# dbdexter-dev/meteor_demod

Measured on AMD Instinct MI355X. Metric: IQ Msamples/s demodulated (whole node), higher is better.
Workload: dtype f32

## Files before the change

### meteor_demod_amd/csrc/demod_device.h

```cpp
#ifndef MDEMOD_DEVICE_H
#define MDEMOD_DEVICE_H

#include <hip/hip_runtime.h>
#include <stdint.h>

#include "pll_flags.h"

#pragma clang fp contract(off)

#define MD_TWO_PI_D 6.283185307179586476925286766559
#define MD_HALF_PI_D 1.5707963267948966192313216916398
#define MD_TWO_PI_F 6.28318548202514648437500f
#define MD_PI_F     3.14159274101257324218750f

struct cf32 { float re, im; };

__device__ __forceinline__ bool md_any(bool p) { return __builtin_amdgcn_ballot_w64(p) != 0ull; }
__device__ __forceinline__ bool md_all(bool p) { return __builtin_amdgcn_ballot_w64(!p) == 0ull; }

template <typename T>
__device__ __forceinline__ T md_lane_select(uint64_t mask, T a, T b)
{
	static_assert(sizeof(T) == 4, "one 32-bit register");
	T r;
// ... 157 lines not shown
	x.re = x.re - bias_re;
	x.im = x.im - bias_im;
	x.re = x.re * gain;
	x.im = x.im * gain;
	return x;
}

template <bool SHORT = false>
__device__ __forceinline__ void
md_agc_gain(cf32 scaled, float &gain)
{
	const float mag = SHORT ? md_cabsf_short(scaled.re, scaled.im) : md_cabsf(scaled.re, scaled.im);
	gain = gain + 0.0001f * (190.0f - mag);
	gain = (0.0f > gain) ? 0.0f : gain;
}

__device__ __forceinline__ float
md_agc_gain_step(float gain, float mag)
{
	gain = gain + 0.0001f * (190.0f - mag);
	return (0.0f > gain) ? 0.0f : gain;
}

template <bool SHORT = false>
__device__ __forceinline__ cf32
md_agc(cf32 x, float &gain, float &bias_re, float &bias_im)
{
	x = md_agc_apply(x, gain, bias_re, bias_im);
	md_agc_gain<SHORT>(x, gain);
	return x;
}

#define MD_TWO_PI_LO (-0x1.777a5cp-23f)

template <bool F32 = false>
__device__ __forceinline__ void
md_nco_advance(float &phase, float freq)
{
	phase = phase + freq;
	if (F32) {
		const float w = (phase - MD_TWO_PI_F) - MD_TWO_PI_LO;
		phase = (phase >= MD_TWO_PI_F) ? w : phase;
	} else if (phase >= MD_TWO_PI_F)
		phase = (float)((double)phase - MD_TWO_PI_D);
}

#define MD_FOUR_PI_F 12.56637096405029296875f
__device__ __forceinline__ float
md_wrap_2pi(float xf)
{
	const bool wraps = !(fabsf(xf) < MD_TWO_PI_F);
	const float once = (xf < 0.0f) ? (xf + MD_TWO_PI_F) + MD_TWO_PI_LO : (xf - MD_TWO_PI_F) - MD_TWO_PI_LO;
	float r = wraps ? once : xf;
	const bool far = !(fabsf(xf) < MD_FOUR_PI_F);
	if (__builtin_expect(md_any(far), 0)) {
		if (far) r = (float)fmod((double)xf, MD_TWO_PI_D);
	}
	return r;
}

__device__ __forceinline__ float
md_wrap_2pi_near(float xf, bool &far)
{
	const bool wraps = !(fabsf(xf) < MD_TWO_PI_F);
	const float once = (xf < 0.0f) ? (xf + MD_TWO_PI_F) + MD_TWO_PI_LO : (xf - MD_TWO_PI_F) - MD_TWO_PI_LO;
	far = !(fabsf(xf) < MD_FOUR_PI_F);
	return wraps ? once : xf;
}
__device__ __forceinline__ float md_wrap_2pi_far(float xf) { return (float)fmod((double)xf, MD_TWO_PI_D); }

__device__ __forceinline__ float
md_tanh_lut(const float *lut, float v)
{
	const float c = __builtin_amdgcn_fmed3f(v, -16.0f, 15.0f);
	return lut[(int)c + 16];
}

__device__ __forceinline__ float
md_tanh_lut_uniform(const float *lut, float v)
{
	float t = (v >= 15.0f) ? 1.0f : -1.0f;
	if (__builtin_expect(md_any(v > -16.0f && v < 15.0f), 0)) t = md_tanh_lut(lut, v);
	return t;
}

__device__ __forceinline__ void
md_tanh_lut_uniform2(const float *lut, float a, float b, float &ta, float &tb)
{
	ta = (a >= 15.0f) ? 1.0f : -1.0f;
	tb = (b >= 15.0f) ? 1.0f : -1.0f;
	if (__builtin_expect(md_any((a > -16.0f && a < 15.0f) || (b > -16.0f && b < 15.0f)), 0)) {
		ta = md_tanh_lut(lut, a);
// ... 67 lines not shown
		if (__builtin_expect((m_lock_event | m_turn) != 0ull, 0)) {
			const PllFlagStep s = pll_flags_step(fl, md_lane_bit(m_below), md_lane_bit(m_above),
			                                     p.freq >= fmax ? PLL_FREQ_HIGH : (p.freq <= -fmax ? PLL_FREQ_LOW : PLL_FREQ_INSIDE));
			fl = s.fl; first = s.first; changed = s.changed;
		}
		p.freq = md_clamp_sym(p.freq, fmax);
		return changed;
	}

	const uint32_t below = (p.err < 85.0f) ? 1u : 0u, above = (p.err > 105.0f) ? 1u : 0u;
	const uint32_t lock_now = below & (fl ^ 1u);
	const uint32_t unlock_now = above & fl;
	const uint32_t lock2 = lock_now + lock_now;
	first = lock2 ^ (lock2 & fl);
	fl = fl | lock_now | lock2;
	fl = fl ^ (fl & unlock_now);

	if (!(fl & 1u)) p.freq = (float)((double)p.freq + ((fl & 4u) ? 0.000001 : -0.000001));
	fl = (p.freq >= fmax) ? (fl & ~4u) : ((p.freq <= -fmax) ? (fl | 4u) : fl);
	p.freq = md_clamp_sym(p.freq, fmax);
	return lock_now | unlock_now;
}

__device__ __forceinline__ uint64_t
md_pll_update_common(PllWord &p, uint32_t fl, const float *lut, float alpha, float beta, float fmax, float i, float q, float &ph, bool &far)
{
	const float ti = md_tanh_lut(lut, i), tq = md_tanh_lut(lut, q);
	const float e = ti * q - tq * i;

	ph = p.phase + alpha * e;
	p.phase = md_wrap_2pi_near(ph, far);
	p.freq = p.freq + beta * e;

	const float decayed = p.err * (1.0f - 0.001f);
	p.err = (float)((double)decayed + fabs((double)e) * (double)0.001f);

	const uint64_t m_below = __builtin_amdgcn_ballot_w64(p.err < 85.0f), m_above = __builtin_amdgcn_ballot_w64(p.err > 105.0f);
	const uint64_t m_locked = __builtin_amdgcn_ballot_w64((fl & 1u) != 0);
	const uint64_t m_lock_event = (m_below & ~m_locked) | (m_above & m_locked);
	const float swept = (float)((double)p.freq + ((fl & 4u) ? 0.000001 : -0.000001));
	p.freq = md_lane_select(m_locked ^ m_lock_event, swept, p.freq);
	const uint64_t m_turn = __builtin_amdgcn_ballot_w64(fabsf(p.freq) >= fmax);
	return m_lock_event | m_turn;
}

__device__ __forceinline__ uint32_t
md_pll_update_rare(const PllWord &p, uint32_t &fl, float fmax, uint32_t &first)
{
	const PllFlagStep s = pll_flags_step(fl, p.err < 85.0f ? 1u : 0u, p.err > 105.0f ? 1u : 0u,
	                                     p.freq >= fmax ? PLL_FREQ_HIGH : (p.freq <= -fmax ? PLL_FREQ_LOW : PLL_FREQ_INSIDE));
	fl = s.fl; first = s.first;
	return s.changed;
}

// ... 25 lines not shown
```

### meteor_demod_amd/csrc/demod_kernel_gat.hip

```cpp
#include "rotwin_body.h"
#include "hip_host.h"

namespace {

typedef float gpair_t __attribute__((ext_vector_type(2)));
typedef float gquad_t __attribute__((ext_vector_type(4)));
typedef __attribute__((address_space(3))) const gquad_t lds_gquad;
typedef __attribute__((address_space(3))) const float lds_gfloat;

template <int FMT> struct GFmt;
template <> struct GFmt<16> {
	enum { G = 4 };
	__device__ static __forceinline__ gpair_t get(const uint4 &q, int k) { const uint32_t w = (&q.x)[k]; return gpair_t{ (float)(int)(int16_t)(w & 0xFFFFu), (float)((int)w >> 16) }; }
	__device__ static __forceinline__ gpair_t one(uint32_t w) { return gpair_t{ (float)(int)(int16_t)(w & 0xFFFFu), (float)((int)w >> 16) }; }
};
template <> struct GFmt<8> {
	enum { G = 8 };
	__device__ static __forceinline__ gpair_t get(const uint4 &q, int k) { const uint32_t w = (&q.x)[k >> 1] >> (16 * (k & 1)); return gpair_t{ (float)((int)(w & 0xFFu) - 128), (float)((int)((w >> 8) & 0xFFu) - 128) }; }
	__device__ static __forceinline__ gpair_t one(uint16_t w) { return gpair_t{ (float)((int)(w & 0xFFu) - 128), (float)((int)(w >> 8) - 128) }; }
};
template <> struct GFmt<32> {
	enum { G = 2 };
	__device__ static __forceinline__ gpair_t get(const uint4 &q, int k) { return gpair_t{ __uint_as_float((&q.x)[2 * k]), __uint_as_float((&q.x)[2 * k + 1]) }; }
	__device__ static __forceinline__ gpair_t one(float2 w) { return gpair_t{ w.x, w.y }; }
};

template <int KT, int FMT>
struct WinG {
	static constexpr int G = GFmt<FMT>::G, kTaps = KT, kBack = KT - 1, AMAX = G - 1, NS = KT + AMAX, NW = 4 * ((NS + 3) / 4), SLIDE = 4, MAXSL = 1, DEPTH = 1,
	                     BLOCK = MDEMOD_RW_BLOCK, ROTN = 1, RING = 32, REGSLOTS = 0;
	static constexpr bool GATHER = true, SCALAR_SLIDE = false, VCONST = false;
	static constexpr bool LOCK_EARLY_OUT = true;
	static constexpr bool RARE_ONE_BRANCH = false;
	static_assert(NS % G == 0 && NS / G <= 36, "whole 16-byte loads, and few enough of them to stay in registers");
	typedef typename RFmt<FMT>::sample_t sample_t;
	__device__ __forceinline__ void setup(uint32_t) {}
	__device__ static __forceinline__ void put_history(const float2 *, bool, int) {}
	__device__ static __forceinline__ void put_init(const RGran<FMT> (&)[1], int) {}
	__device__ static __forceinline__ void put(const RGran<FMT> (&)[1], int) {}
	__device__ static __forceinline__ void fir(uint32_t, int, int, const DemodConsts &, int, float &, float &) {}

	__device__ static __forceinline__ void
	fir_gather(uint32_t ctab_addr, const sample_t *src, const float2 *hist, int v, int n, int bank, const DemodConsts &C, float &re, float &im)
	{
		const int oldest = v - kBack - (KT - 1);
		const int d = oldest & (G - 1);
		const int start = oldest - d;
		const int o = AMAX - d;
		const uint32_t row = ctab_addr + 4u * (uint32_t)(__mul24(bank * 4 + (o & 3), C.ctab_row_stride) + (o & ~3));
		gpair_t acc = { 0.0f, 0.0f };
		if (__builtin_expect(md_all(start >= 0 && start + NS <= n), 1)) {
			uint4 raw[NS / G];
#pragma unroll
			for (int g = 0; g < NS / G; g++) __builtin_memcpy(&raw[g], src + start + G * g, 16);
#pragma unroll
			for (int s4 = 0; s4 < NS / 4; s4++) {
// ... 74 lines not shown
```

### meteor_demod_amd/csrc/demod_kernel_rot.hip

```cpp
#include "rotwin_body.h"
#include "rot_fir_bounds.h"
#include "hip_host.h"
#ifdef ROTWIN_ASM_HEADER
#include ROTWIN_ASM_HEADER
#else
#include "rotwin_asm.h"
#endif

namespace {

static_assert(ROTWIN_NCH * 8 == 80 && ROTWIN_SLIDE == 8, "window = ten chunks of eight, a slide brings one");


__device__ __forceinline__ void
rot_fir(uint32_t row_addr, int rot, int flags, float &re, float &im)
{
	int tmp;
#if ROTWIN_PK == 1 || ROTWIN_PK == 3
	typedef float pair_t __attribute__((ext_vector_type(2)));
	pair_t acc, p0, p1;
	asm volatile(ROTWIN_FIR_ASM
	             : [acc] "=&v"(acc), [p0] "=&v"(p0), [p1] "=&v"(p1), [tmp] "=&s"(tmp)
	             : [addr] "v"(row_addr), [rot] "s"(rot), [flags] "s"(flags)
	             : "vcc", "scc", ROTWIN_COEF_CLOBBERS);
// ... 33 lines not shown
{
	int tmp;
	asm volatile(ROTWIN_PUT_F32_ASM
	             : [tmp] "=&s"(tmp), [rot] "+s"(q), [base] "+s"(base)
	             : [f0] "v"(f[0]), [f1] "v"(f[1]), [f2] "v"(f[2]), [f3] "v"(f[3]), [f4] "v"(f[4]), [f5] "v"(f[5]), [f6] "v"(f[6]), [f7] "v"(f[7]),
	               [f8] "v"(f[8]), [f9] "v"(f[9]), [f10] "v"(f[10]), [f11] "v"(f[11]), [f12] "v"(f[12]), [f13] "v"(f[13]), [f14] "v"(f[14]), [f15] "v"(f[15])
	             : "vcc", "scc", "v255", "memory");
}
__device__ __forceinline__ void
rot_put_floats(const uint32_t (&f)[16], int q)
{
	int base = 0;
	rot_put_floats(f, q, base);
}
template <> __device__ __forceinline__ void
rot_put<32>(const RGran<32> &a, const RGran<32> &b, int &q, int &base)
{
	uint32_t f[16];
#pragma unroll
	for (int i = 0; i < 8; i++) { f[i] = a.w[i]; f[8 + i] = b.w[i]; }
	rot_put_floats(f, q, base);
}

template <int FMT, int COMPACT = 0, int BLK = MDEMOD_RW_BLOCK, int VC = 0, int RSL = 0>
struct WinF {
	static constexpr int kTaps = 65, kBack = 64, NW = 80, SLIDE = 8, AMAX = NW - kTaps, MAXSL = 1, DEPTH = 1, BLOCK = BLK, ROTN = NW / SLIDE, RING = 32;
	static constexpr bool GATHER = false;
	static constexpr bool SCALAR_SLIDE = true;
	static constexpr bool VCONST = VC != 0;
	static_assert(SLIDE == ROTWIN_SLIDE && ROTN == ROTWIN_NCH, "the slide's assembly counts for itself");
	__device__ __forceinline__ void setup(uint32_t) {}
	static constexpr int REGSLOTS = RSL;
	static constexpr bool LOCK_EARLY_OUT = true;
	static constexpr bool RARE_ONE_BRANCH = true;
	__device__ static __forceinline__ void put_history(const float2 *hist, bool valid, int q)
	{
		const uint4 *h4 = reinterpret_cast<const uint4 *>(hist);
		uint32_t f[16];
#pragma unroll
		for (int i = 0; i < 4; i++) {
			uint4 h = h4[i];
			if (!valid) h = make_uint4(0, 0, 0, 0);
			f[4 * i] = h.x; f[4 * i + 1] = h.y; f[4 * i + 2] = h.z; f[4 * i + 3] = h.w;
		}
		rot_put_floats(f, q);
	}
	__device__ static __forceinline__ void put(const RGran<FMT> (&g)[2], int q) { int base = 0; rot_put<FMT>(g[0], g[1], q, base); }
	__device__ static __forceinline__ void put_init(const RGran<FMT> (&g)[2], int q) { put(g, q); }
	__device__ static __forceinline__ void slide(const RGran<FMT> (&g)[2], int &rot, int &base) { rot_put<FMT>(g[0], g[1], rot, base); }
	__device__ static __forceinline__ void fir(uint32_t ctab_addr, int a, int bank, const DemodConsts &C, int rot, float &re, float &im)
	{
		const int o = AMAX - a;
		uint32_t row_addr;
		if (COMPACT) row_addr = rot_mad24((uint32_t)(bank * 4 + (o & 3)), 4u * (uint32_t)C.ctab_row_stride, ctab_addr + 4u * (uint32_t)(o & ~3));
		else row_addr = rot_mad24(rot_mad24((uint32_t)a, (uint32_t)C.interp, (uint32_t)bank), 4u * (uint32_t)C.ctab_row_stride, ctab_addr);
		static_assert(AMAX == 15, "two bits of a / 4");
		const uint64_t ex = __builtin_amdgcn_ballot_w64(true);
		const RotFirQ q = rot_fir_q(ex, __builtin_amdgcn_ballot_w64(a >= 4), __builtin_amdgcn_ballot_w64(a >= 8), __builtin_amdgcn_ballot_w64(a >= 12));
		int q_hi = q.q_hi;
		asm("" : "+s"(q_hi));
		const int flags = rot_fir_flags(q.q_lo, q_hi);
#ifdef ROT_EXP_NOSKIP
		int f0 = __builtin_amdgcn_readfirstlane(flags);
		asm volatile("s_and_b32 %0, %0, 0" : "+s"(f0) : : "scc");
		rot_fir(row_addr, rot, f0, re, im);
#else
		rot_fir(row_addr, rot, flags, re, im);
#endif
	}
};

typedef float pair_t2 __attribute__((ext_vector_type(2)));

template <int NA>
__device__ __forceinline__ void
rot_fir_acc(uint32_t addr, int rot, int last, pair_t2 &acc)
{
	int tmp;
// ... 28 lines not shown
	else
		asm volatile(ROTWIN_MIGRATE5_ASM : [tmp] "=&s"(tmp) : ROT_F16_OPERANDS, [rot] "s"(q) : "vcc", "scc", "v255", ROTWIN_ACC_CLOBBERS, "memory");
}
template <int NA>
__device__ __forceinline__ void
rot_put_acc(const uint32_t (&f)[16], int q)
{
	int tmp;
	if constexpr (NA == 10)
		asm volatile(ROTWIN_PUT_ACC_ASM : [tmp] "=&s"(tmp) : ROT_F16_OPERANDS, [rot] "s"(q) : "vcc", "scc", ROTWIN_ACC_CLOBBERS, "memory");
	else if constexpr (NA == 2)
		asm volatile(ROTWIN_PUT_ACC2_ASM : [tmp] "=&s"(tmp) : ROT_F16_OPERANDS, [rot] "s"(q) : "vcc", "scc", ROTWIN_ACC_CLOBBERS, "memory");
	else
		asm volatile(ROTWIN_PUT_ACC5_ASM : [tmp] "=&s"(tmp) : ROT_F16_OPERANDS, [rot] "s"(q) : "vcc", "scc", ROTWIN_ACC_CLOBBERS, "memory");
}

template <int BLK, int NA, int MSL>
struct WinH {
	static constexpr int NR = 10, SLIDE = 8, NW = SLIDE * (NR + NA), kTaps = NA == 10 ? 129 : 65, kBack = kTaps - 1, AMAX = NW - kTaps, MAXSL = MSL, DEPTH = MSL,
	                     BLOCK = BLK, ROTN = NR, RING = 32, REGSLOTS = 0;
	static constexpr bool GATHER = false, SCALAR_SLIDE = false, VCONST = false;
	static constexpr bool LOCK_EARLY_OUT = true;
	static constexpr bool RARE_ONE_BRANCH = false;
	static_assert((NA == 10 || NA == 2 || NA == 5) && AMAX == (NA == 5 ? 55 : 31) && kBack % SLIDE == 0, "wide (160 slots, 129 taps), mid (96 slots, 65 taps) or far (120 slots, 65 taps)");
	__device__ __forceinline__ void setup(uint32_t) {}
	__device__ static __forceinline__ void place(const uint32_t (&f)[16], int c)
	{
		if (c < NR) rot_put_floats(f, c);
		else rot_put_acc<NA>(f, c - NR);
	}
	__device__ static __forceinline__ void put_history(const float2 *hist, bool valid, int c)
	{
		const uint4 *h4 = reinterpret_cast<const uint4 *>(hist);
		uint32_t f[16];
#pragma unroll
		for (int i = 0; i < 4; i++) {
			uint4 h = h4[i];
			if (!valid) h = make_uint4(0, 0, 0, 0);
			f[4 * i] = h.x; f[4 * i + 1] = h.y; f[4 * i + 2] = h.z; f[4 * i + 3] = h.w;
		}
		place(f, c);
	}
	__device__ static __forceinline__ void put_init(const RGran<32> (&g)[2], int c)
	{
		uint32_t f[16];
#pragma unroll
// ... 99 lines not shown
```

### meteor_demod_amd/csrc/demod_kernel_rotp.hip

```cpp
#include "rotwin_body.h"
#include "hip_host.h"
#ifdef ROTPK_ASM_HEADER
#include ROTPK_ASM_HEADER
#else
#include "rotpk_asm.h"
#endif

namespace {

typedef float pair_t __attribute__((ext_vector_type(2)));

template <int GEO> struct GeoP;
#ifndef ROTP_WIDE_DEPTH
#define ROTP_WIDE_DEPTH 1
#endif
#ifndef ROTP_MID_DEPTH
#define ROTP_MID_DEPTH 1
#endif
#ifndef ROTP_FAR_DEPTH
#define ROTP_FAR_DEPTH 2
#endif
template <> struct GeoP<0> { static constexpr int kTaps = 129, NW = MDEMOD_RW_WIDE_NW, MAXSL = 1, DEPTH = ROTP_WIDE_DEPTH, BLOCK = MDEMOD_RW_WIDE_BLOCK; };
template <> struct GeoP<1> { static constexpr int kTaps = 65, NW = MDEMOD_RW_MID_NW, MAXSL = 1, DEPTH = ROTP_MID_DEPTH, BLOCK = MDEMOD_RW_BLOCK; };
#ifndef ROTP_FAR_MAXSL
// ... 37 lines not shown
		               [g7] "v"(g[7]), [g8] "v"(g[8]), [g9] "v"(g[9]), [g10] "v"(g[10]), [g11] "v"(g[11]), [g12] "v"(g[12]),  \
		               [g13] "v"(g[13]), [g14] "v"(g[14]), [g15] "v"(g[15]), [rot] "s"(q)                                     \
		             : "vcc", "scc", "v255", "memory");                                                                       \
	}
#define ROTP_PUT8(GEO, NAME)                                                                                                  \
	__device__ __forceinline__ void AsmP<GEO, 8>::put(const uint32_t (&g)[8], int q)                                          \
	{                                                                                                                         \
		int tmp;                                                                                                              \
		asm volatile(ROTPK_##NAME##_8_PUT_ASM                                                                                 \
		             : [tmp] "=&s"(tmp)                                                                                       \
		             : [g0] "v"(g[0]), [g1] "v"(g[1]), [g2] "v"(g[2]), [g3] "v"(g[3]), [g4] "v"(g[4]), [g5] "v"(g[5]), [g6] "v"(g[6]),  \
		               [g7] "v"(g[7]), [rot] "s"(q)                                                                           \
		             : "vcc", "scc", "v255", "memory");                                                                       \
	}
ROTP_PUT16(0, WIDE) ROTP_PUT16(1, MID) ROTP_PUT16(2, FAR) ROTP_PUT8(0, WIDE) ROTP_PUT8(1, MID) ROTP_PUT8(2, FAR)

template <int GEO, int FMT>
struct WinP {
	static constexpr int kTaps = GeoP<GEO>::kTaps, kBack = kTaps - 1, NW = GeoP<GEO>::NW, SLIDE = 16, AMAX = NW - kTaps,
	                     MAXSL = GeoP<GEO>::MAXSL, DEPTH = GeoP<GEO>::DEPTH, BLOCK = GeoP<GEO>::BLOCK, NCH = NW / SLIDE, GD = FMT == 16 ? 16 : 8, REGSLOTS = 0, ROTN = NCH, RING = 32;
	static constexpr bool GATHER = false, SCALAR_SLIDE = false, VCONST = false;
	static constexpr bool LOCK_EARLY_OUT = true;
	static constexpr bool RARE_ONE_BRANCH = false;
	__device__ __forceinline__ void setup(uint32_t) {}
	static_assert(kBack % SLIDE == 0 && NW % SLIDE == 0, "history and window are whole chunks");

	__device__ static __forceinline__ void put_history(const float2 *hist, bool valid, int q)
	{
		uint32_t g[GD];
#pragma unroll
		for (int k = 0; k < 16; k++) {
			float2 h = hist[k];
			if (!valid) h = make_float2(0.0f, 0.0f);
			if (FMT == 16) {
				g[k] = ((uint32_t)(int)h.x & 0xFFFFu) | ((uint32_t)(int)h.y << 16);
			} else {
				const uint32_t s = (uint32_t)(((int)h.x + 128) & 0xFF) | ((uint32_t)(((int)h.y + 128) & 0xFF) << 8);
				if (k & 1) g[k / 2] |= s << 16; else g[k / 2] = s;
			}
		}
		AsmP<GEO, FMT>::put(g, q);
	}
	__device__ static __forceinline__ void put(const RGran<FMT> (&gr)[4], int q)
	{
		uint32_t g[GD];
#pragma unroll
// ... 65 lines not shown
```

### meteor_demod_amd/csrc/rot_firing_index.h

```cpp
#ifndef MDEMOD_ROT_FIRING_INDEX_H
#define MDEMOD_ROT_FIRING_INDEX_H

#include <stdint.h>

#if defined(__HIPCC__) || defined(__CUDACC__)
#define ROT_IDX_HD __host__ __device__
#else
#define ROT_IDX_HD
#endif


ROT_IDX_HD constexpr bool
rot_ring_geometry_ok(uint32_t ring, uint32_t block)
{
	return (ring == 16u || ring == 32u) && (block == 256u || block == 512u);
}

ROT_IDX_HD constexpr uint32_t
rot_ring_group_bytes(uint32_t block)
{
	return block * 16u;
}

ROT_IDX_HD constexpr uint32_t
// ... 27 lines not shown
}


enum { ROT_CLOCK_ROW_SHIFT = 6 };

ROT_IDX_HD constexpr uint32_t
rot_clock_sel(bool c1, bool c2, bool c3)
{
	return c1 ? 0u : (c2 ? 16u : (c3 ? 32u : 48u));
}

ROT_IDX_HD constexpr int32_t
rot_clock_entry_scaled(int32_t isub)
{
	return (int32_t)((uint32_t)isub << ROT_CLOCK_ROW_SHIFT);
}

ROT_IDX_HD constexpr int32_t
rot_clock_entry_unscaled(int32_t isub_scaled)
{
	return isub_scaled >> ROT_CLOCK_ROW_SHIFT;
}

#endif
```

### meteor_demod_amd/csrc/rotwin_body.h

```cpp
#ifndef MDEMOD_ROTWIN_BODY_H
#define MDEMOD_ROTWIN_BODY_H

#include <hip/hip_runtime.h>
#include <stdint.h>

#include "demod_internal.h"
#include "demod_device.h"
#include "clock_jump.h"
#include "rot_firing_index.h"

#pragma clang fp contract(off)

#ifndef ROT_OQ_SYNC
#define ROT_OQ_SYNC 1
#endif
typedef float rot_sinlut_t;

namespace {

template <int FMT> struct RFmt;
template <> struct RFmt<16> { typedef uint32_t sample_t; enum { GDW = 4 }; };
template <> struct RFmt<8>  { typedef uint16_t sample_t; enum { GDW = 2 }; };
template <> struct RFmt<32> { typedef float2   sample_t; enum { GDW = 8 }; };

// ... 20 lines not shown
}

__device__ __forceinline__ uint32_t
rot_mad24(uint32_t a, uint32_t b, uint32_t c)
{
	uint32_t r;
	asm("v_mad_u32_u24 %0, %1, %2, %3" : "=v"(r) : "v"(a), "s"(b), "v"(c));
	return r;
}

template <int K>
__device__ __forceinline__ float
blind_steps(float p, float f)
{
#pragma unroll
	for (int k = 0; k < K; k++) p = p + f;
	return p;
}

template <int KS> struct RotIsub { enum { SHIFT = KS == 109 ? 0 : ROT_CLOCK_ROW_SHIFT, ONE = 1 << SHIFT }; };
typedef int rot_i4 __attribute__((ext_vector_type(4)));
typedef const __attribute__((address_space(3))) rot_i4 *rot_clktab_t;
struct RotClockConsts { int k_safe, steps_need, interp; float f_hi; uint32_t magic; float inv; const cj_sched *jump; rot_clktab_t tab; };
template <int KS>
__device__ __forceinline__ void
rot_clock_fast(const RotClockConsts &K, float thr, int v_end, int v_fast_end, float &t_phase, float t_freq, int &isub, int &v_cur, int &bank, bool &fired, int jidx = -1)
{
	int k_safe = KS ? KS : K.k_safe;
	const int interp = K.interp;
	const bool jump = KS == 0 && jidx >= 0 && K.jump[jidx < 0 ? 0 : jidx].nb > 0;
	const cj_sched &J = K.jump[jidx < 0 ? 0 : jidx];
	const bool fast = (KS == 109 ? (t_phase > CJ109_P_LO && t_phase < CJ109_P_HI)
	                   : jump    ? (t_phase > J.floor && t_phase < J.hi)
	                             : (t_phase < thr - (float)k_safe * K.f_hi - 1e-3f))
	                  && (jump ? (v_cur + J.need < v_end) : (v_cur < v_fast_end));
	if (fast) {
		float p = t_phase;
		if (KS == 109) k_safe = clock_jump_109(p, t_freq, thr, K.inv);
		else if (KS) p = blind_steps<KS>(p, t_freq);
		else if (jump) k_safe = clock_jump_run(p, t_freq, thr, K.f_hi, K.inv, J);
		else {
			int k = k_safe;
			for (; k >= 16; k -= 16) p = blind_steps<16>(p, t_freq);
			if (k & 8) p = blind_steps<8>(p, t_freq);
			if (k & 4) p = blind_steps<4>(p, t_freq);
			if (k & 2) p = blind_steps<2>(p, t_freq);
			if (k & 1) p = p + t_freq;
		}
		const float p1 = p + t_freq, p2 = p1 + t_freq, p3 = p2 + t_freq, p4 = p3 + t_freq;
		const bool c1 = p1 >= thr, c2 = p2 >= thr, c3 = p3 >= thr, c4 = p4 >= thr;
		float ph = c3 ? p3 : p4;
		ph = c2 ? p2 : ph;
		ph = c1 ? p1 : ph;
		t_phase = ph;
		if ((KS == 14 || KS == 6) || (KS == 0 && K.tab)) {
			const uint32_t off = (uint32_t)isub + rot_clock_sel(c1, c2, c3);
			const rot_i4 e = *reinterpret_cast<rot_clktab_t>(reinterpret_cast<const __attribute__((address_space(3))) unsigned char *>(K.tab) + off);
			v_cur += e.x;
			isub = e.z;
			bank = e.w;
		} else {
			const int isub_old = isub >> RotIsub<KS>::SHIFT;
			const uint32_t w = (uint32_t)(isub_old + k_safe + 1 + (c1 ? 0 : 1) + (c2 ? 0 : 1) + (c3 ? 0 : 1));
			const uint32_t q = (interp == 1) ? w : __umulhi(w, K.magic);
			const int isub_new = (int)(w - q * (uint32_t)interp);
			v_cur += (int)q + (isub_new > 0 ? 1 : 0) - (isub_old > 0 ? 1 : 0);
			const int fire_sub = (isub_new == 0) ? interp - 1 : isub_new - 1;
			bank = interp - 1 - fire_sub;
			isub = isub_new << RotIsub<KS>::SHIFT;
		}
		fired = c4;
	}
}


template <class W, int FMT, int OQPSK, int KS, int LUT = 0>
__device__ __forceinline__ void
rotwin_demod(const DemodLaunch &L)
{
	typedef typename RFmt<FMT>::sample_t sample_t;
	constexpr int kBack = W::kBack, SLIDE = W::SLIDE, AMAX = W::AMAX, BLOCK = W::BLOCK, NCH = W::NW / W::SLIDE, GPS = W::SLIDE / 4;
	constexpr int NST = GPS * W::DEPTH;
	static_assert(W::DEPTH >= W::MAXSL, "a loop iteration may slide MAXSL times");
	constexpr int ROTN = W::ROTN, RING = W::RING, RGR = RING / 8;
	constexpr bool GATHER = W::GATHER;
	static_assert(RING == 32 || RING == 16, "output ring");
	constexpr int RS = W::REGSLOTS;
#ifndef ROT_PRIO
#define ROT_PRIO 1
#endif
#ifndef ROT_PRIO_LEVEL
#define ROT_PRIO_LEVEL 2
#endif
	constexpr bool RARE = W::RARE_ONE_BRANCH;
	constexpr int PRIO = ROT_PRIO;

	extern __shared__ __attribute__((aligned(16))) unsigned char lds[];
	float *ctab = reinterpret_cast<float *>(lds);
	float *lut = ctab + L.ctab_floats;
	enum { S_GAIN, S_BIAS_RE, S_BIAS_IM, S_PHASE, S_FREQ, S_ERR, S_FLAGS, S_TPREV, S_INPHASE, S_EVCALL, S_FIRSTLOCK, S_LASTV, S_COUNT };
	static_assert(S_COUNT == MDEMOD_RW_STATE_SLOTS, "host LDS sizing");
	uint32_t sl_addr = (uint32_t)(uintptr_t)(__attribute__((address_space(3))) unsigned char *)lds
	                   + 4u * (L.ctab_floats + 32u + (threadIdx.x >> 6) * (uint32_t)(S_COUNT * 64) + (threadIdx.x & 63u));
	asm("" : "+v"(sl_addr));
	float *sl = (float *)(__attribute__((address_space(3))) float *)(uintptr_t)sl_addr;
	int *sli = reinterpret_cast<int *>(sl);
	uint4 *stage = reinterpret_cast<uint4 *>(lut + 32 + (BLOCK / 64) * (S_COUNT * 64)) + threadIdx.x;
	const uint32_t ctab_addr = (uint32_t)(uintptr_t)(__attribute__((address_space(3))) unsigned char *)lds;
	W win;
	rot_sinlut_t *sintab = reinterpret_cast<rot_sinlut_t *>(stage - threadIdx.x + BLOCK * RGR);
	if constexpr (LUT) md_sin_lut_fill(sintab, (int)threadIdx.x, BLOCK);
	win.setup(ctab_addr + (uint32_t)(reinterpret_cast<unsigned char *>(stage - threadIdx.x + BLOCK * RGR) - lds) + (LUT ? MDEMOD_SIN_LUT_BYTES : 0));
	rot_i4 *clktab = reinterpret_cast<rot_i4 *>(reinterpret_cast<unsigned char *>(stage - threadIdx.x + BLOCK * RGR) + (LUT ? MDEMOD_SIN_LUT_BYTES : 0));

	const DemodConsts &C = L.c;
	const uint32_t stream = blockIdx.x * blockDim.x + threadIdx.x;
	const bool valid = stream < L.n_streams;

	for (uint32_t i = threadIdx.x; i < L.ctab_floats; i += blockDim.x) ctab[i] = L.ctab[i];
	if (threadIdx.x < 32) lut[threadIdx.x] = L.tanh_lut[threadIdx.x];
	const bool has_clktab = KS != 109 && C.clock_tab != nullptr;
	if (has_clktab)
		for (int i = (int)threadIdx.x; i < 4 * C.interp; i += (int)blockDim.x) {
			rot_i4 e = reinterpret_cast<const rot_i4 *>(C.clock_tab)[i];
			e.z = rot_clock_entry_scaled(e.z);
			clktab[i] = e;
		}

	int n = 0;
	const sample_t *src = nullptr;
	if (valid) {
		n = (int)(L.n_samples_arr ? L.n_samples_arr[stream] : L.n_samples);
		const uint64_t off = L.iq_offset ? L.iq_offset[stream] : (uint64_t)stream * L.iq_stride;
		src = reinterpret_cast<const sample_t *>(L.iq) + off;
	}
	const int v_end = kBack + n;
	const int interp = C.interp;

	float t_phase = 0.0f, t_freq = C.t_center;
	int dual_state = 1;
	float r_gain = 1.0f, r_bias_re = 0.0f, r_bias_im = 0.0f, r_phase = 0.0f, r_freq = 0.0f;
	float r_err = 1000.0f, r_tprev = 0.0f;
	int r_flags = 0, r_lastv = -1;
	auto ld_err = [&]() -> float { return (RS & 1) ? r_err : sl[S_ERR * 64]; };
	auto st_err = [&](float v) { if (RS & 1) r_err = v; else sl[S_ERR * 64] = v; };
	auto ld_tprev = [&]() -> float { return (RS & 2) ? r_tprev : sl[S_TPREV * 64]; };
	auto st_tprev = [&](float v) { if (RS & 2) r_tprev = v; else sl[S_TPREV * 64] = v; };
// ... 31 lines not shown
		for (int c = 0; c < NCH - kBack / SLIDE; c++) {
			RGran<FMT> g[GPS];
#pragma unroll
			for (int i = 0; i < GPS; i++) g[i] = rot_fetch<FMT>(src, SLIDE * c + 4 * i, n);
			win.put_init(g, __builtin_amdgcn_readfirstlane(kBack / SLIDE + c));
		}
	}
	int g_load = (W::NW - kBack) / 4;
	RGran<FMT> stg[GATHER ? 1 : NST];
	if constexpr (!GATHER) {
#pragma unroll
		for (int i = 0; i < NST; i++) stg[i] = rot_fetch<FMT>(src, 4 * (g_load + i), n);
		g_load += NST;
	}

	__syncthreads();

	int rot = 0;
	int slot = 1;
	int base = 0;
	if constexpr (W::SCALAR_SLIDE) asm("s_mov_b32 %0, 0\n\ts_mov_b32 %1, 0" : "=s"(rot), "=s"(base));
	int isub = 0, bank = interp - 1;
	constexpr int ISH = RotIsub<KS>::SHIFT, IONE = RotIsub<KS>::ONE;
	bool fired = false;
	bool done = !valid || n == 0;
	constexpr int V_DONE = 0x3FFFFFFF;
	int v_cur = done ? V_DONE : kBack - 1;
	static_assert(rot_ring_geometry_ok(RING, BLOCK), "output ring: the offset's two fields");
	uint32_t ring_off = 0;
	auto sym_count = [&]() -> uint32_t { return ld_symbase() + rot_ring_count(ring_off, BLOCK); };
	RotClockConsts K;
	K.k_safe = C.step_safe; K.f_hi = C.step_fmax; K.magic = C.interp_magic; K.interp = C.interp; K.inv = C.step_inv;
	K.steps_need = ((KS == 109 ? CJ109_MAX_STEPS : C.step_safe) + 4 + C.interp - 1) / C.interp;
	K.jump = C.jump;
	K.tab = has_clktab ? (rot_clktab_t)clktab : (rot_clktab_t)0;
	const int v_fast_end = v_end - K.steps_need;
	float k_t_alpha = C.t_alpha, k_t_beta = C.t_beta, k_t_center = C.t_center, k_pll_alpha = C.pll_alpha, k_pll_beta = C.pll_beta;
	if constexpr (W::VCONST) asm("" : "+v"(k_t_alpha), "+v"(k_t_beta), "+v"(k_t_center), "+v"(k_pll_alpha), "+v"(k_pll_beta));

	int n_wave_max = n;
	for (int o = 32; o > 0; o >>= 1) {
		const int other = __shfl_xor(n_wave_max, o);
		n_wave_max = other > n_wave_max ? other : n_wave_max;
	}
	n_wave_max = __builtin_amdgcn_readfirstlane(n_wave_max);
	const uint64_t guard64 = 4ull * (uint64_t)(n_wave_max + kBack) * (uint64_t)interp + 4096ull;
	uint32_t guard = guard64 > 0xFFFFFFFFull ? 0xFFFFFFFFu : (uint32_t)guard64;
#ifdef ROT_EXP_TIMING
	uint64_t tacc[5] = { 0, 0, 0, 0, 0 }, tlast = clock64();
	uint32_t n_iter = 0, n_fir = 0, n_slide = 0, n_wslow = 0;
#define ROT_TICK(i) do { const uint64_t t_ = clock64(); tacc[i] += t_ - tlast; tlast = t_; } while (0)
#else
#define ROT_TICK(i) do { } while (0)
#endif
	do {
		ROT_TICK(4);
		if (!fired && !done) {
			const float thr = OQPSK ? (float)dual_state * MD_PI_F : MD_TWO_PI_F;
			rot_clock_fast<KS>(K, thr, v_end, v_fast_end, t_phase, t_freq, isub, v_cur, bank, fired);
			while (!fired && !done) {
				if (isub == 0) {
					if (v_cur + 1 >= v_end) { done = true; v_cur = V_DONE; break; }
					v_cur++;
				}
				t_phase = t_phase + t_freq;
				bank = interp - 1 - (isub >> ISH);
				isub = (isub + IONE == (interp << ISH)) ? 0 : isub + IONE;
				if (t_phase >= thr) fired = true;
			}
		}
		if constexpr (GATHER) if (md_all(v_cur == V_DONE)) break;
		ROT_TICK(0);
#ifdef ROT_EXP_TIMING
		n_iter++;
#endif

		bool all_done = false;
		if constexpr (!GATHER)
#pragma unroll
		for (int r = 0; r < W::MAXSL; r++) {
			const int a_now = v_cur - kBack - base;
			if (md_all(a_now >= SLIDE)) {
				if (md_all(v_cur == V_DONE)) { all_done = true; break; }
				RGran<FMT> g[GPS];
#pragma unroll
				for (int i = 0; i < GPS; i++) g[i] = stg[i];
				if constexpr (W::SCALAR_SLIDE) win.slide(g, rot, base);
				else {
					win.put(g, __builtin_amdgcn_readfirstlane(rot));
					rot = __builtin_amdgcn_readfirstlane((rot == ROTN - 1) ? 0 : rot + 1);
					base = __builtin_amdgcn_readfirstlane(base + SLIDE);
				}
#pragma unroll
				for (int i = 0; i + GPS < NST; i++) stg[i] = stg[i + GPS];
				const int m_new = 4 * g_load;
				if (md_all(m_new + SLIDE - 1 < n)) {
#pragma unroll
					for (int i = 0; i < GPS; i++) __builtin_memcpy(&stg[NST - GPS + i], src + m_new + 4 * i, sizeof(RGran<FMT>));
				} else {
#pragma unroll
					for (int i = 0; i < GPS; i++) stg[NST - GPS + i] = rot_fetch<FMT>(src, m_new + 4 * i, n);
				}
				g_load += GPS;
			}
		}
		if (all_done) break;

		ROT_TICK(1);
		const int a = v_cur - kBack - base;
		if (fired && (GATHER || a <= AMAX) && (!(OQPSK && ROT_OQ_SYNC) || dual_state == slot)) {
			fired = false;
			cf32 y;
			if constexpr (GATHER) win.fir_gather(ctab_addr, src, hist_in, v_cur, n, bank, C, y.re, y.im);
			else win.fir(ctab_addr, a, bank, C, W::SCALAR_SLIDE ? rot : __builtin_amdgcn_readfirstlane(rot), y.re, y.im);
			if (PRIO) __builtin_amdgcn_s_setprio(ROT_PRIO_LEVEL);
			ROT_TICK(2);
#ifdef ROT_EXP_TIMING
			n_fir++;
#endif

			constexpr bool SHORT_ABS = KS == 14 && !OQPSK && LUT;
			float mag = 0.0f;
			uint64_t m_abs = 0;
			if constexpr (RARE && SHORT_ABS) {
				y = md_agc_apply(y, r_gain, r_bias_re, r_bias_im);
				mag = md_cabsf_short_try(y.re, y.im, m_abs);
			} else y = md_agc<SHORT_ABS>(y, r_gain, r_bias_re, r_bias_im);
			uint32_t fl = (uint32_t)ld_flags();
			PllWord pll;
			pll.phase = r_phase; pll.freq = r_freq;
			pll.err = ld_err();

			float sn, cs;
			if constexpr (LUT) {
				sn = md_sin_from_code_lut(sintab, md_turn_code<false>(-pll.phase));
				cs = md_sin_from_code_lut(sintab, md_turn_code<false>((float)((double)(-pll.phase) + MD_HALF_PI_D)));
			} else {
				sn = md_fast_sin<false>(-pll.phase);
				cs = md_fast_cos<false>(-pll.phase);
			}
			bool emit = true;
			float out_re, out_im;
			if (OQPSK) {
				float inphase = sl[S_INPHASE * 64];
				const int rail = ROT_OQ_SYNC ? slot : dual_state;
				if (rail == 1) { inphase = y.re * cs - y.im * sn; emit = false; sl[S_INPHASE * 64] = inphase; }
				out_re = inphase;
				out_im = y.re * sn + y.im * cs;
				dual_state = 3 - rail;
// ... 3 lines not shown
			}
			md_nco_advance<true>(pll.phase, pll.freq);

			uint64_t m_again = 0;
			auto ring_back = [&]() {
				const uint32_t prev = sym_count() - 1u;
				st_symbase(prev & ~(uint32_t)(RING - 1));
				ring_off = rot_ring_off(prev, RING, BLOCK);
			};
			if (emit) {
				const bool again = (v_cur == ld_lastv());
				if constexpr (RARE) { m_again = __builtin_amdgcn_ballot_w64(again); asm volatile("" : "+s"(m_again)); }
				int lastv = v_cur;
				if constexpr ((RS & 8) != 0) asm("" : "+v"(lastv));
				st_lastv(lastv);
				if constexpr (!RARE)
					if (__builtin_expect(md_any(again), 0)) {
						if (again) ring_back();
					}
				float t_prev = ld_tprev();
				md_timing_update(t_phase, t_freq, t_prev, k_t_alpha, k_t_beta, k_t_center, C.t_maxdev, out_im);
				st_tprev(t_prev);
			}
			rot_clock_fast<KS>(K, OQPSK ? (float)dual_state * MD_PI_F : MD_TWO_PI_F, v_end, v_fast_end, t_phase, t_freq, isub, v_cur, bank, fired,
			                   OQPSK ? (ROT_OQ_SYNC ? 2 - slot : -1) : 0);
#ifdef ROT_EXP_TIMING
			if (!fired) n_slide++;
			if (md_any(!fired)) n_wslow++;
#endif
			if (emit) {
				uint32_t first = 0;
				auto lock_event = [&](uint32_t fl_now) {
					const uint32_t sym_now = sym_count();
					if (first) sli[S_FIRSTLOCK * 64] = (int)sym_now;
					const int ev_call = sli[S_EVCALL * 64];
					if (ev_call < MDEMOD_MAX_LOCK_EVENTS) {
						mdemod_lock_event ev;
						ev.symbol = L.st.n_symbols[stream] + sym_now; ev.locked = (int)(fl_now & 1u); ev.pad = 0;
						L.st.events[(size_t)stream * MDEMOD_MAX_LOCK_EVENTS + ev_call] = ev;
					}
					sli[S_EVCALL * 64] = ev_call + 1;
				};
				if constexpr (RARE) {
					float ph;
					bool far;
					const uint64_t m_pll = md_pll_update_common(pll, fl, lut, k_pll_alpha, k_pll_beta, C.pll_fmax, out_re, out_im, ph, far);
					const uint64_t rare = m_pll | __builtin_amdgcn_ballot_w64(far) | m_again | m_abs;
					if (__builtin_expect(rare != 0ull, 0)) {
						if (md_lane_bit(m_abs)) mag = md_cabsf_exact(y.re, y.im);
						if (md_lane_bit(m_again)) ring_back();
						if (far) pll.phase = md_wrap_2pi_far(ph);
						uint32_t fl_new = fl;
						if (md_pll_update_rare(pll, fl_new, C.pll_fmax, first)) lock_event(fl_new);
						asm volatile("v_mov_b32 %0, %1" : "+v"(fl) : "v"(fl_new));
					}
					pll.freq = md_clamp_sym(pll.freq, C.pll_fmax);
					if constexpr (SHORT_ABS) r_gain = md_agc_gain_step(r_gain, mag);
				} else {
					const uint32_t changed = md_pll_update_packed<false, W::LOCK_EARLY_OUT>(pll,fl, lut, k_pll_alpha, k_pll_beta, C.pll_fmax, out_re, out_im, first);
					if (__builtin_expect(changed != 0, 0)) lock_event(fl);
				}
				const uint32_t sym = (uint32_t)(md_quantise(out_re) & 0xFF) | ((uint32_t)(md_quantise(out_im) & 0xFF) << 8);
				*reinterpret_cast<uint16_t *>(reinterpret_cast<unsigned char *>(stage) + ring_off) = (uint16_t)sym;
				ring_off = rot_ring_step(ring_off, RING, BLOCK);
				asm volatile("" : "+v"(r_gain), "+v"(pll.err));
				if (__builtin_expect(ring_off == 0, 0)) {
					const uint32_t sym_call = ld_symbase() + (uint32_t)RING;
					st_symbase(sym_call);
					int8_t *soft_out = L.soft + (size_t)stream * L.soft_stride * 2;
					if (__builtin_expect(sym_call <= L.soft_cap, 1)) {
						int8_t *dst = soft_out + 2 * (size_t)(sym_call - RING);
#pragma unroll
						for (int g4 = 0; g4 < RGR; g4++) {
							const uint4 qv = stage[g4 * BLOCK];
							__builtin_memcpy(dst + 16 * g4, &qv, 16);
							asm volatile("" ::: "memory");
						}
					} else {
						fl |= 8;
						for (uint32_t i = 0; i < (uint32_t)RING && sym_call - RING + i < L.soft_cap; i++)
// ... 80 lines not shown
```

Baseline: 290,800.

## Carry FIR row address incrementally and simplify wrap and AGC clamp

Adds a PLAIN_ADDS policy, on by default (7) for the WinF rotating-window kernel, that turns on three changes. The phase wrap uses a magnitude-and-copysign form in place of the sign-tested select. The AGC gain clamp becomes fmaxf. The FIR coefficient-table row address is carried incrementally through precomputed per-entry row steps in the clock table, replacing the nested mad24 recomputation each symbol. These aim to cut VALU instructions on the per-symbol critical path. In exchange the clock-table setup gets more complex, and fmaxf treats NaN differently from the old select.

```diff
diff --git a/meteor_demod_amd/csrc/demod_device.h b/meteor_demod_amd/csrc/demod_device.h
--- a/meteor_demod_amd/csrc/demod_device.h
+++ b/meteor_demod_amd/csrc/demod_device.h
@@ -203,6 +203,13 @@
 	return (0.0f > gain) ? 0.0f : gain;
 }
 
+__device__ __forceinline__ float
+md_agc_gain_step_max(float gain, float mag)
+{
+	gain = gain + 0.0001f * (190.0f - mag);
+	return __builtin_fmaxf(gain, 0.0f);
+}
+
 template <bool SHORT = false>
 __device__ __forceinline__ cf32
 md_agc(cf32 x, float &gain, float &bias_re, float &bias_im)
@@ -249,6 +256,25 @@
 	return wraps ? once : xf;
 }
 __device__ __forceinline__ float md_wrap_2pi_far(float xf) { return (float)fmod((double)xf, MD_TWO_PI_D); }
+
+__device__ __forceinline__ float
+md_wrap_2pi_near_bfi(float xf, bool &far)
+{
+	const bool wraps = !(fabsf(xf) < MD_TWO_PI_F);
+	const float s_hi = __builtin_copysignf(MD_TWO_PI_F, xf), s_lo = __builtin_copysignf(-MD_TWO_PI_LO, xf);
+	const float once = (xf - s_hi) + s_lo;
+	far = !(fabsf(xf) < MD_FOUR_PI_F);
+	return wraps ? once : xf;
+}
+__device__ __forceinline__ float
+md_wrap_2pi_near_mag(float xf, bool &far)
+{
+	const bool wraps = !(fabsf(xf) < MD_TWO_PI_F);
+	const float w = (fabsf(xf) - MD_TWO_PI_F) - MD_TWO_PI_LO;
+	const float once = __builtin_copysignf(w, xf);
+	far = !(fabsf(xf) < MD_FOUR_PI_F);
+	return wraps ? once : xf;
+}
 
 __device__ __forceinline__ float
 md_tanh_lut(const float *lut, float v)
@@ -362,6 +388,7 @@
 	return lock_now | unlock_now;
 }
 
+template <int WRAP = 0>
 __device__ __forceinline__ uint64_t
 md_pll_update_common(PllWord &p, uint32_t fl, const float *lut, float alpha, float beta, float fmax, float i, float q, float &ph, bool &far)
 {
@@ -369,7 +396,7 @@
 	const float e = ti * q - tq * i;
 
 	ph = p.phase + alpha * e;
-	p.phase = md_wrap_2pi_near(ph, far);
+	p.phase = WRAP == 1 ? md_wrap_2pi_near_mag(ph, far) : WRAP == 2 ? md_wrap_2pi_near_bfi(ph, far) : md_wrap_2pi_near(ph, far);
 	p.freq = p.freq + beta * e;
 
 	const float decayed = p.err * (1.0f - 0.001f);
diff --git a/meteor_demod_amd/csrc/demod_kernel_gat.hip b/meteor_demod_amd/csrc/demod_kernel_gat.hip
--- a/meteor_demod_amd/csrc/demod_kernel_gat.hip
+++ b/meteor_demod_amd/csrc/demod_kernel_gat.hip
@@ -32,6 +32,7 @@
 	static constexpr bool GATHER = true, SCALAR_SLIDE = false, VCONST = false;
 	static constexpr bool LOCK_EARLY_OUT = true;
 	static constexpr bool RARE_ONE_BRANCH = false;
+	static constexpr int PLAIN_ADDS = 0;
 	static_assert(NS % G == 0 && NS / G <= 36, "whole 16-byte loads, and few enough of them to stay in registers");
 	typedef typename RFmt<FMT>::sample_t sample_t;
 	__device__ __forceinline__ void setup(uint32_t) {}
diff --git a/meteor_demod_amd/csrc/demod_kernel_rot.hip b/meteor_demod_amd/csrc/demod_kernel_rot.hip
--- a/meteor_demod_amd/csrc/demod_kernel_rot.hip
+++ b/meteor_demod_amd/csrc/demod_kernel_rot.hip
@@ -79,6 +79,10 @@
 	rot_put_floats(f, q, base);
 }
 
+#ifndef ROT_PLAIN_ADDS
+#define ROT_PLAIN_ADDS 7
+#endif
+
 template <int FMT, int COMPACT = 0, int BLK = MDEMOD_RW_BLOCK, int VC = 0, int RSL = 0>
 struct WinF {
 	static constexpr int kTaps = 65, kBack = 64, NW = 80, SLIDE = 8, AMAX = NW - kTaps, MAXSL = 1, DEPTH = 1, BLOCK = BLK, ROTN = NW / SLIDE, RING = 32;
@@ -90,6 +94,7 @@
 	static constexpr int REGSLOTS = RSL;
 	static constexpr bool LOCK_EARLY_OUT = true;
 	static constexpr bool RARE_ONE_BRANCH = true;
+	static constexpr int PLAIN_ADDS = ROT_PLAIN_ADDS;
 	__device__ static __forceinline__ void put_history(const float2 *hist, bool valid, int q)
 	{
 		const uint4 *h4 = reinterpret_cast<const uint4 *>(hist);
@@ -111,6 +116,10 @@
 		uint32_t row_addr;
 		if (COMPACT) row_addr = rot_mad24((uint32_t)(bank * 4 + (o & 3)), 4u * (uint32_t)C.ctab_row_stride, ctab_addr + 4u * (uint32_t)(o & ~3));
 		else row_addr = rot_mad24(rot_mad24((uint32_t)a, (uint32_t)C.interp, (uint32_t)bank), 4u * (uint32_t)C.ctab_row_stride, ctab_addr);
+		fir_at(row_addr, a, rot, re, im);
+	}
+	__device__ static __forceinline__ void fir_at(uint32_t row_addr, int a, int rot, float &re, float &im)
+	{
 		static_assert(AMAX == 15, "two bits of a / 4");
 		const uint64_t ex = __builtin_amdgcn_ballot_w64(true);
 		const RotFirQ q = rot_fir_q(ex, __builtin_amdgcn_ballot_w64(a >= 4), __builtin_amdgcn_ballot_w64(a >= 8), __builtin_amdgcn_ballot_w64(a >= 12));
@@ -185,6 +194,7 @@
 	static constexpr bool GATHER = false, SCALAR_SLIDE = false, VCONST = false;
 	static constexpr bool LOCK_EARLY_OUT = true;
 	static constexpr bool RARE_ONE_BRANCH = false;
+	static constexpr int PLAIN_ADDS = 0;
 	static_assert((NA == 10 || NA == 2 || NA == 5) && AMAX == (NA == 5 ? 55 : 31) && kBack % SLIDE == 0, "wide (160 slots, 129 taps), mid (96 slots, 65 taps) or far (120 slots, 65 taps)");
 	__device__ __forceinline__ void setup(uint32_t) {}
 	__device__ static __forceinline__ void place(const uint32_t (&f)[16], int c)
diff --git a/meteor_demod_amd/csrc/demod_kernel_rotp.hip b/meteor_demod_amd/csrc/demod_kernel_rotp.hip
--- a/meteor_demod_amd/csrc/demod_kernel_rotp.hip
+++ b/meteor_demod_amd/csrc/demod_kernel_rotp.hip
@@ -83,6 +83,7 @@
 	static constexpr bool GATHER = false, SCALAR_SLIDE = false, VCONST = false;
 	static constexpr bool LOCK_EARLY_OUT = true;
 	static constexpr bool RARE_ONE_BRANCH = false;
+	static constexpr int PLAIN_ADDS = 0;
 	__device__ __forceinline__ void setup(uint32_t) {}
 	static_assert(kBack % SLIDE == 0 && NW % SLIDE == 0, "history and window are whole chunks");
 
diff --git a/meteor_demod_amd/csrc/rot_firing_index.h b/meteor_demod_amd/csrc/rot_firing_index.h
--- a/meteor_demod_amd/csrc/rot_firing_index.h
+++ b/meteor_demod_amd/csrc/rot_firing_index.h
@@ -73,4 +73,41 @@
 	return isub_scaled >> ROT_CLOCK_ROW_SHIFT;
 }
 
+
+ROT_IDX_HD constexpr int32_t
+rot_clock_bank_of(int32_t isub, int32_t interp)
+{
+	return isub == 0 ? 0 : interp - isub;
+}
+
+ROT_IDX_HD constexpr uint32_t
+rot_row_addr(int32_t a, int32_t bank, int32_t interp, uint32_t stride, uint32_t base)
+{
+	return (uint32_t)(a * interp + bank) * stride + base;
+}
+
+ROT_IDX_HD constexpr uint32_t
+rot_row_step(int32_t advance, int32_t bank_new, int32_t isub_old, int32_t interp, uint32_t stride)
+{
+	return (uint32_t)(advance * interp + bank_new - rot_clock_bank_of(isub_old, interp)) * stride;
+}
+
+ROT_IDX_HD constexpr uint32_t
+rot_row_slide(int32_t slide, int32_t interp, uint32_t stride)
+{
+	return (uint32_t)(slide * interp) * stride;
+}
+
+ROT_IDX_HD constexpr int32_t
+rot_clock_entry_row_step(int32_t index, int32_t advance, int32_t bank_new, int32_t interp, uint32_t stride)
+{
+	return (int32_t)rot_row_step(advance, bank_new, index >> 2, interp, stride);
+}
+
+ROT_IDX_HD constexpr int32_t
+rot_clock_entry_fire_sub(int32_t bank_new, int32_t interp)
+{
+	return interp - 1 - bank_new;
+}
+
 #endif
diff --git a/meteor_demod_amd/csrc/rotwin_body.h b/meteor_demod_amd/csrc/rotwin_body.h
--- a/meteor_demod_amd/csrc/rotwin_body.h
+++ b/meteor_demod_amd/csrc/rotwin_body.h
@@ -66,9 +66,12 @@
 typedef int rot_i4 __attribute__((ext_vector_type(4)));
 typedef const __attribute__((address_space(3))) rot_i4 *rot_clktab_t;
 struct RotClockConsts { int k_safe, steps_need, interp; float f_hi; uint32_t magic; float inv; const cj_sched *jump; rot_clktab_t tab; };
-template <int KS>
+template <bool ON> struct RotRow;
+template <> struct RotRow<false> { __device__ __forceinline__ void step(int) {} };
+template <> struct RotRow<true> { uint32_t addr; __device__ __forceinline__ void step(int by) { addr += (uint32_t)by; } };
+template <int KS, bool ROWC = false>
 __device__ __forceinline__ void
-rot_clock_fast(const RotClockConsts &K, float thr, int v_end, int v_fast_end, float &t_phase, float t_freq, int &isub, int &v_cur, int &bank, bool &fired, int jidx = -1)
+rot_clock_fast(const RotClockConsts &K, float thr, int v_end, int v_fast_end, float &t_phase, float t_freq, int &isub, int &v_cur, int &bank, bool &fired, int jidx, RotRow<ROWC> &row)
 {
 	int k_safe = KS ? KS : K.k_safe;
 	const int interp = K.interp;
@@ -103,6 +106,7 @@
 			v_cur += e.x;
 			isub = e.z;
 			bank = e.w;
+			row.step(e.y);
 		} else {
 			const int isub_old = isub >> RotIsub<KS>::SHIFT;
 			const uint32_t w = (uint32_t)(isub_old + k_safe + 1 + (c1 ? 0 : 1) + (c2 ? 0 : 1) + (c3 ? 0 : 1));
@@ -137,6 +141,9 @@
 #define ROT_PRIO_LEVEL 2
 #endif
 	constexpr bool RARE = W::RARE_ONE_BRANCH;
+	constexpr int PLAIN = W::PLAIN_ADDS;
+	constexpr bool ROWC = (PLAIN & 4) != 0 && (KS == 14 || KS == 6);
+	static_assert(!(PLAIN & 9) || RARE, "the wrap without the sign test is a form of the rare-path policy's near wrap");
 	constexpr int PRIO = ROT_PRIO;
 
 	extern __shared__ __attribute__((aligned(16))) unsigned char lds[];
@@ -167,6 +174,7 @@
 	if (has_clktab)
 		for (int i = (int)threadIdx.x; i < 4 * C.interp; i += (int)blockDim.x) {
 			rot_i4 e = reinterpret_cast<const rot_i4 *>(C.clock_tab)[i];
+			if constexpr (ROWC) e.y = rot_clock_entry_row_step(i, e.x, e.w, C.interp, 4u * (uint32_t)C.ctab_row_stride);
 			e.z = rot_clock_entry_scaled(e.z);
 			clktab[i] = e;
 		}
@@ -244,6 +252,8 @@
 	if constexpr (W::SCALAR_SLIDE) asm("s_mov_b32 %0, 0\n\ts_mov_b32 %1, 0" : "=s"(rot), "=s"(base));
 	int isub = 0, bank = interp - 1;
 	constexpr int ISH = RotIsub<KS>::SHIFT, IONE = RotIsub<KS>::ONE;
+	RotRow<ROWC> row;
+	if constexpr (ROWC) row.addr = 0;
 	bool fired = false;
 	bool done = !valid || n == 0;
 	constexpr int V_DONE = 0x3FFFFFFF;
@@ -279,7 +289,7 @@
 		ROT_TICK(4);
 		if (!fired && !done) {
 			const float thr = OQPSK ? (float)dual_state * MD_PI_F : MD_TWO_PI_F;
-			rot_clock_fast<KS>(K, thr, v_end, v_fast_end, t_phase, t_freq, isub, v_cur, bank, fired);
+			rot_clock_fast<KS, ROWC>(K, thr, v_end, v_fast_end, t_phase, t_freq, isub, v_cur, bank, fired, -1, row);
 			while (!fired && !done) {
 				if (isub == 0) {
 					if (v_cur + 1 >= v_end) { done = true; v_cur = V_DONE; break; }
@@ -290,6 +300,8 @@
 				isub = (isub + IONE == (interp << ISH)) ? 0 : isub + IONE;
 				if (t_phase >= thr) fired = true;
 			}
+			if constexpr (ROWC)
+				row.addr = rot_mad24(rot_mad24((uint32_t)(v_cur - kBack - base), (uint32_t)interp, (uint32_t)rot_clock_bank_of(isub >> ISH, interp)), 4u * (uint32_t)C.ctab_row_stride, ctab_addr);
 		}
 		if constexpr (GATHER) if (md_all(v_cur == V_DONE)) break;
 		ROT_TICK(0);
@@ -313,6 +325,7 @@
 					rot = __builtin_amdgcn_readfirstlane((rot == ROTN - 1) ? 0 : rot + 1);
 					base = __builtin_amdgcn_readfirstlane(base + SLIDE);
 				}
+				if constexpr (ROWC) row.addr -= rot_row_slide(SLIDE, interp, 4u * (uint32_t)C.ctab_row_stride);
 #pragma unroll
 				for (int i = 0; i + GPS < NST; i++) stg[i] = stg[i + GPS];
 				const int m_new = 4 * g_load;
@@ -334,6 +347,7 @@
 			fired = false;
 			cf32 y;
 			if constexpr (GATHER) win.fir_gather(ctab_addr, src, hist_in, v_cur, n, bank, C, y.re, y.im);
+			else if constexpr (ROWC) win.fir_at(row.addr, a, rot, y.re, y.im);
 			else win.fir(ctab_addr, a, bank, C, W::SCALAR_SLIDE ? rot : __builtin_amdgcn_readfirstlane(rot), y.re, y.im);
 			if (PRIO) __builtin_amdgcn_s_setprio(ROT_PRIO_LEVEL);
 			ROT_TICK(2);
@@ -347,6 +361,9 @@
 			if constexpr (RARE && SHORT_ABS) {
 				y = md_agc_apply(y, r_gain, r_bias_re, r_bias_im);
 				mag = md_cabsf_short_try(y.re, y.im, m_abs);
+			} else if constexpr ((PLAIN & 2) != 0 && !SHORT_ABS) {
+				y = md_agc_apply(y, r_gain, r_bias_re, r_bias_im);
+				r_gain = md_agc_gain_step_max(r_gain, md_cabsf(y.re, y.im));
 			} else y = md_agc<SHORT_ABS>(y, r_gain, r_bias_re, r_bias_im);
 			uint32_t fl = (uint32_t)ld_flags();
 			PllWord pll;
@@ -396,8 +413,8 @@
 				md_timing_update(t_phase, t_freq, t_prev, k_t_alpha, k_t_beta, k_t_center, C.t_maxdev, out_im);
 				st_tprev(t_prev);
 			}
-			rot_clock_fast<KS>(K, OQPSK ? (float)dual_state * MD_PI_F : MD_TWO_PI_F, v_end, v_fast_end, t_phase, t_freq, isub, v_cur, bank, fired,
-			                   OQPSK ? (ROT_OQ_SYNC ? 2 - slot : -1) : 0);
+			rot_clock_fast<KS, ROWC>(K, OQPSK ? (float)dual_state * MD_PI_F : MD_TWO_PI_F, v_end, v_fast_end, t_phase, t_freq, isub, v_cur, bank, fired,
+			                         OQPSK ? (ROT_OQ_SYNC ? 2 - slot : -1) : 0, row);
 #ifdef ROT_EXP_TIMING
 			if (!fired) n_slide++;
 			if (md_any(!fired)) n_wslow++;
@@ -418,7 +435,7 @@
 				if constexpr (RARE) {
 					float ph;
 					bool far;
-					const uint64_t m_pll = md_pll_update_common(pll, fl, lut, k_pll_alpha, k_pll_beta, C.pll_fmax, out_re, out_im, ph, far);
+					const uint64_t m_pll = md_pll_update_common<(PLAIN & 1) ? 1 : (PLAIN & 8) ? 2 : 0>(pll, fl, lut, k_pll_alpha, k_pll_beta, C.pll_fmax, out_re, out_im, ph, far);
 					const uint64_t rare = m_pll | __builtin_amdgcn_ballot_w64(far) | m_again | m_abs;
 					if (__builtin_expect(rare != 0ull, 0)) {
 						if (md_lane_bit(m_abs)) mag = md_cabsf_exact(y.re, y.im);
@@ -429,7 +446,7 @@
 						asm volatile("v_mov_b32 %0, %1" : "+v"(fl) : "v"(fl_new));
 					}
 					pll.freq = md_clamp_sym(pll.freq, C.pll_fmax);
-					if constexpr (SHORT_ABS) r_gain = md_agc_gain_step(r_gain, mag);
+					if constexpr (SHORT_ABS) r_gain = (PLAIN & 2) ? md_agc_gain_step_max(r_gain, mag) : md_agc_gain_step(r_gain, mag);
 				} else {
 					const uint32_t changed = md_pll_update_packed<false, W::LOCK_EARLY_OUT>(pll,fl, lut, k_pll_alpha, k_pll_beta, C.pll_fmax, out_re, out_im, first);
 					if (__builtin_expect(changed != 0, 0)) lock_event(fl);
```

Result: no change. 291,400, median of 6 (+0.2%).
